# PaddlePaddle/PGL

Hardware: AMD Instinct MI355X
Metric: aggregated edges/sec (GCN send+recv_sum, d=128) (higher is better)
Workload: dtype f32

## Files before the change

pgl_amd/csrc/aggregate.hip:

```cpp
#include "aggregate_flat.hpp"
#include "aggregate_dense2.hpp"

namespace pglamd {

int chunk_edges() {
    static int k = [] {
        const char* s = getenv("PGLAMD_CHUNK");
        int v = s ? atoi(s) : 256;
        if (v < 8) v = 8;
        return v / 8 * 8;
    }();
    return k;
}

int chunk_edges_for(int64_t num_edges) {
    if (getenv("PGLAMD_CHUNK")) return chunk_edges();
    return num_edges >= 12000000 ? 256 : num_edges >= 5000000 ? 128 : 64;
}

ProfileState& prof() { static ProfileState s; return s; }

int32_t launch_fixup_cols(const AggParams& p, int32_t dtype, int rcls, hipStream_t st) {
#define PGLAMD_FIXUP(T) (rcls == 0 ? launch_fixups<T, 1, 1, 0>(p, st) : launch_fixups<T, 1, 1, 1>(p, st))
    switch (dtype) {
// ... 57 lines not shown
    PGLAMD_LAUNCH_CHECK();
    return PGLAMD_OK;
}

template int32_t aggregate_typed<float>(PGLAMD_AGG_ARGS);
extern template int32_t aggregate_typed<double>(PGLAMD_AGG_ARGS);
extern template int32_t aggregate_typed<int32_t>(PGLAMD_AGG_ARGS);
extern template int32_t aggregate_typed<int64_t>(PGLAMD_AGG_ARGS);
extern template int32_t aggregate_typed<__half>(PGLAMD_AGG_ARGS);
extern template int32_t aggregate_typed<__hip_bfloat16>(PGLAMD_AGG_ARGS);

}

using namespace pglamd;

extern "C" size_t pglamd_aggregate_workspace_bytes(int64_t num_edges, int64_t dout, int32_t dtype) {
    size_t es = dtype_size(dtype);
    if (es == 0 || num_edges <= 0) return 256;
    int64_t k = chunk_edges_for(num_edges);
    if ((int64_t)(dout * (int64_t)es) <= group_row_bytes()) k = std::min<int64_t>(k, group_chunk_edges(16));
    const int64_t n_chunks = ceil_div(num_edges, k);
    const int64_t max_cols = 1024;
    const int64_t tile = dout < max_cols ? dout : max_cols;
    if (es == 2) es = 4;
    return SplitWs(n_chunks, tile, es).bytes() + 256;
}

static int32_t aggregate_entry(const void* x, int32_t dtype, int64_t dx, const void* y, int64_t dy, const int32_t* eid,
                               const int32_t* row, const int32_t* col, const int64_t* indptr, int64_t num_edges,
                               int64_t n_csr_rows, int64_t out_rows, int64_t dout, int32_t message_op, int32_t reduce_op,
                               const float* src_scale, const float* dst_scale, int32_t accumulate, void* out, void* workspace,
                               size_t workspace_bytes, const AggExtra& ex, void* stream) {
    if (!out || !indptr || (num_edges > 0 && (!x || !row))) return fail(PGLAMD_E_ARG, "aggregate: NULL pointer");
    if (num_edges < 0 || num_edges > kMaxEdges || n_csr_rows >= INT32_MAX || out_rows >= INT32_MAX)
        return fail(PGLAMD_E_RANGE, "aggregate: sizes beyond int32 engine range");
    if (dout <= 0 || dx <= 0 || dout % dx != 0 || (y && (dy <= 0 || dout % dy != 0)))
        return fail(PGLAMD_E_SHAPE, "aggregate: dx=%lld dy=%lld dout=%lld is not a trailing-dim broadcast",
                    (long long)dx, (long long)dy, (long long)dout);
    if (reduce_op < 0 || reduce_op > 3 || (y && (message_op < 0 || message_op > 3)))
        return fail(PGLAMD_E_ARG, "aggregate: bad op enum");
    if (ex.x2 && (ex.x_split < 0 || ex.x_split >= INT32_MAX)) return fail(PGLAMD_E_RANGE, "aggregate_ext: x_split out of range");
    hipStream_t st = static_cast<hipStream_t>(stream);
#define CALL(T) aggregate_typed<T>(x, dx, y, dy, eid, row, col, indptr, num_edges, n_csr_rows, out_rows, dout, \
                                   message_op, reduce_op, src_scale, dst_scale, accumulate, out, workspace, workspace_bytes, ex, st)
    switch (dtype) {
        case PGLAMD_F32: return CALL(float);
        case PGLAMD_F64: return CALL(double);
        case PGLAMD_I32: return CALL(int32_t);
        case PGLAMD_I64: return CALL(int64_t);
        case PGLAMD_F16: return CALL(__half);
        case PGLAMD_BF16: return CALL(__hip_bfloat16);
        default: return fail(PGLAMD_E_DTYPE, "aggregate: dtype %d not supported", dtype);
    }
#undef CALL
}

extern "C" int32_t pglamd_aggregate(const void* x, int32_t dtype, int64_t n_x_rows, int64_t dx, const void* y,
                                    int64_t dy, const int32_t* eid, const int32_t* row, const int32_t* col,
                                    const int64_t* indptr, int64_t num_edges, int64_t n_csr_rows,
                                    int64_t out_rows, int64_t dout, int32_t message_op, int32_t reduce_op,
                                    const float* src_scale, const float* dst_scale, int32_t accumulate, void* out,
                                    void* workspace, size_t workspace_bytes, void* stream) {
    (void)n_x_rows;
    return aggregate_entry(x, dtype, dx, y, dy, eid, row, col, indptr, num_edges, n_csr_rows, out_rows, dout, message_op, reduce_op,
                           src_scale, dst_scale, accumulate, out, workspace, workspace_bytes, AggExtra{}, stream);
}

extern "C" int32_t pglamd_aggregate_ext(const void* x, const void* x2, int64_t x_split, int32_t dtype, int64_t dx, int64_t ldx,
                                        const void* y, int64_t dy, const int32_t* eid, const int32_t* row, const int32_t* col,
                                        const int64_t* indptr, const int64_t* zero_indptr, int64_t max_row_edges,
                                        int64_t num_edges, int64_t n_csr_rows, int64_t out_rows, int64_t dout, int64_t ldout,
                                        int32_t message_op, int32_t reduce_op, const float* dst_scale, int32_t accumulate,
                                        void* out, void* workspace, size_t workspace_bytes, int32_t flags, void* stream) {
    if (ldx < 0 || ldout < 0) return fail(PGLAMD_E_ARG, "aggregate_ext: negative row stride");
    if (flags & ~PGLAMD_AGG_DEAL_CHUNKS) return fail(PGLAMD_E_ARG, "aggregate_ext: unknown flag bits 0x%x", (unsigned)flags);
    AggExtra ex;
    ex.x2 = x2; ex.x_split = x_split; ex.zero_indptr = zero_indptr; ex.max_row_edges = max_row_edges; ex.ldx = ldx; ex.ldo = ldout;
    ex.flags = flags;
    return aggregate_entry(x, dtype, dx, y, dy, eid, row, col, indptr, num_edges, n_csr_rows, out_rows, dout, message_op, reduce_op,
                           nullptr, dst_scale, accumulate, out, workspace, workspace_bytes, ex, stream);
}

namespace pglamd {
template <int VEC>
__global__ __launch_bounds__(kBlock) void agg_slice_combine_kernel(const int* __restrict__ long_rows, int n_long, const float* __restrict__ part,
                                                                  float* __restrict__ out, int d) {
    using V = VecT<float, VEC>;
    const int lane = threadIdx.x & (kWave - 1);
    const int i = wave_uniform((int)blockIdx.x * kWavesPerBlock + (threadIdx.x >> 6));
    if (i >= n_long) return;
    const int r = as_const(long_rows)[i];
    for (int j = lane * VEC; j < d; j += kWave * VEC) {
        float* dst = out + (int64_t)r * d + j;
        V acc = *reinterpret_cast<const V*>(dst);
        V v[kXcds];
#pragma unroll
        for (int s = 0; s < kXcds; ++s) v[s] = *reinterpret_cast<const V*>(part + ((int64_t)s * n_long + i) * d + j);
#pragma unroll
        for (int k = 0; k < VEC; ++k) {
            double a = acc.v[k];
#pragma unroll
            for (int s = 0; s < kXcds; ++s) a += (double)v[s].v[k];
            acc.v[k] = (float)a;
        }
        *reinterpret_cast<V*>(dst) = acc;
    }
}

struct SlicedWs {
    size_t table, part;
    SplitWs split;
    SlicedWs(int64_t n_chunks, int64_t d, int64_t n_hubs, int64_t n_long)
        : table(align_up((size_t)n_hubs * d * sizeof(float), 256)), part(align_up((size_t)kXcds * n_long * d * sizeof(float), 256)),
          split(n_chunks, d, sizeof(float)) {}
    size_t bytes() const { return table + part + split.bytes(); }
};
}

extern "C" size_t pglamd_aggregate_sliced_workspace_bytes(int64_t num_edges, int64_t d, int64_t n_hubs, int64_t n_long, int32_t chunk) {
    if (num_edges <= 0 || d <= 0 || n_hubs < 0 || n_long < 0 || chunk < 8) return 256;
    return SlicedWs(ceil_div(num_edges, chunk), d, n_hubs, n_long).bytes() + 256;
}

extern "C" int32_t pglamd_aggregate_sliced(const float* x, int64_t n_x_rows, int64_t d, const int32_t* hub_ids, int64_t n_hubs,
                                           const int32_t* row, const int32_t* col, const int64_t* indptr, int64_t num_edges,
                                           int64_t out_rows, const int32_t* long_rows, int64_t n_long, const int32_t* blocks,
                                           const int32_t* blocks_dev, int32_t chunk, float* out, void* workspace,
                                           size_t workspace_bytes, void* stream) {
    if (!x || !hub_ids || !row || !col || !indptr || !long_rows || !blocks || !blocks_dev || !out || !workspace)
        return fail(PGLAMD_E_ARG, "aggregate_sliced: NULL pointer");
    const int64_t n_rows = out_rows + kXcds * n_long;
    if (num_edges <= 0 || num_edges > kMaxEdges || n_x_rows <= 0 || n_hubs <= 0 || n_long <= 0 || out_rows <= 0 ||
        n_rows >= INT32_MAX || n_x_rows + n_hubs >= INT32_MAX)
        return fail(PGLAMD_E_RANGE, "aggregate_sliced: sizes beyond int32 engine range");
    if (chunk < 8 || chunk % 8 != 0) return fail(PGLAMD_E_ARG, "aggregate_sliced: chunk %d is not a positive multiple of 8", (int)chunk);
    const int vec = (d % 4 == 0 && d > 128) ? 4 : 2;
    if (d % vec != 0 || d / vec > kWave) return fail(PGLAMD_E_SHAPE, "aggregate_sliced: d = %lld is not an even width up to 128 or a multiple of 4 up to 256", (long long)d);
    if ((reinterpret_cast<uintptr_t>(x) | reinterpret_cast<uintptr_t>(out) | reinterpret_cast<uintptr_t>(workspace)) % (vec * sizeof(float)) != 0)
        return fail(PGLAMD_E_ARG, "aggregate_sliced: x / out / workspace must be %d-byte aligned", (int)(vec * sizeof(float)));
    const int64_t n_chunks = ceil_div(num_edges, chunk), nb = ceil_div(n_chunks, kWavesPerBlock);
    for (int s = 0; s <= kXcds; ++s) {
        const int64_t end = s < kXcds ? blocks[s + 1] : nb;
        if (blocks[s] < 0 || blocks[kXcds + 1 + s] < 0 || (int64_t)blocks[s] + blocks[kXcds + 1 + s] != end || (s == 0 && blocks[0] != 0))
            return fail(PGLAMD_E_ARG, "aggregate_sliced: block table does not tile the %lld blocks of the stream (segment %d)", (long long)nb, s);
    }
    const SlicedWs lay(n_chunks, d, n_hubs, n_long);
    if (workspace_bytes < lay.bytes() + 256) return fail(PGLAMD_E_WORKSPACE, "aggregate_sliced: workspace %zu < %zu", workspace_bytes, lay.bytes() + 256);
    hipStream_t st = static_cast<hipStream_t>(stream);
    char* ws = static_cast<char*>(workspace);
    float* table = reinterpret_cast<float*>(ws);
    float* part = reinterpret_cast<float*>(ws + lay.table);
    PGLAMD_TRY(pglamd_gather_rows(x, d, sizeof(float), hub_ids, 0, n_hubs, table, stream));
    AggParams p{};
    p.x = x; p.x2 = table - n_x_rows * d; p.x_split = (int)n_x_rows;
    p.out = out; p.pout = part - out_rows * d; p.slice_tab = blocks_dev;
    p.row = row; p.col = col; p.indptr = indptr; p.zero_indptr = indptr;
    p.ldx = d; p.ldo = d; p.out_rows = out_rows; p.n_csr_rows = n_rows; p.E = (int)num_edges;
    p.gy = 1; p.j_base = 0; p.tile_cols = (int)d; p.zvec = vec; p.align = 1;
    p.chunk = chunk; p.n_chunks = (int)n_chunks;
    lay.split.carve(p, ws + lay.table + lay.part);
    const int64_t per_xcd = slice_blocks_per_xcd(blocks);
    PGLAMD_TRY(vec == 4 ? launch_flat_sliced<4>(p, per_xcd, st) : launch_flat_sliced<2>(p, per_xcd, st));
    const unsigned grid = (unsigned)ceil_div(n_long, kWavesPerBlock);
    if (vec == 4) hipLaunchKernelGGL(agg_slice_combine_kernel<4>, dim3(grid), dim3(kBlock), 0, st, long_rows, (int)n_long, part, out, (int)d);
    else hipLaunchKernelGGL(agg_slice_combine_kernel<2>, dim3(grid), dim3(kBlock), 0, st, long_rows, (int)n_long, part, out, (int)d);
    PGLAMD_LAUNCH_CHECK();
    return PGLAMD_OK;
}

namespace pglamd {
__global__ __launch_bounds__(kBlock) void pack_weight_kernel(const float* __restrict__ w, int d_in, int d_out, float* __restrict__ wp) {
    const int KK = d_in / 4;
    const int64_t total = (int64_t)(d_out / 16) * KK * kWave;
    for (int64_t i = (int64_t)blockIdx.x * kBlock + threadIdx.x; i < total; i += (int64_t)gridDim.x * kBlock) {
        const int lane = (int)(i % kWave);
        const int64_t t = i / kWave;
        const int kk = (int)(t % KK), ct = (int)(t / KK);
        wp[i] = w[(int64_t)(4 * kk + lane / 16) * d_out + ct * 16 + (lane & 15)];
    }
}

template <int VEC, int SS = 0>
static int32_t launch_dense(AggParams p, hipStream_t st) {
    const int64_t nb = ceil_div(p.n_chunks, kWavesPerBlock);
    p.n_blocks = (int)nb;
    p.n_grid_chunks = (int)xcd_grid(nb);
    const int64_t zb = ceil_div(ceil_div(p.out_rows, kWave), kWavesPerBlock);
    const bool fixups = needs_fixups(p);
    if (fixups) PGLAMD_TRY(reset_split_counters(p, st));
    ProfileScope timed(st, [] { return std::string("agg_flat_kernel<float, ") + (VEC == 2 ? "2" : "1") + ", 1, 0, 0, dense sink>"; });
    hipLaunchKernelGGL((agg_flat_kernel<float, VEC, 1, 0, 0, SS, true, 0, 1>), dim3((unsigned)(p.n_grid_chunks + zb)), dim3(kBlock), 0, st, p);
    PGLAMD_LAUNCH_CHECK();
    PGLAMD_TRY(timed.close());
    if (!fixups) return PGLAMD_OK;
    PGLAMD_TRY((launch_fixups<float, VEC, 1, 0>(p, st)));
    return launch_dense_hub<VEC>(p, st);
}
}

extern "C" size_t pglamd_aggregate_dense_workspace_bytes(int64_t num_edges, int64_t d_in, int64_t d_out) {
    return pglamd_aggregate_workspace_bytes(num_edges, d_in, PGLAMD_F32) + align_up((size_t)(d_in > 0 ? d_in : 1) * (size_t)(d_out > 0 ? d_out : 1) * 4, 256) + 256;
}

extern "C" int32_t pglamd_aggregate_dense(const float* x, int64_t d_in, const int32_t* row, const int32_t* col, const int64_t* indptr,
                                          int64_t num_edges, int64_t n_csr_rows, int64_t out_rows, int32_t reduce_op,
                                          const float* edge_scale, const float* dst_scale, const float* w, const float* bias, int32_t act,
                                          int64_t d_out, float* agg_out, float* out, void* workspace, size_t workspace_bytes, void* stream) {
    if (!out || !w || !indptr || (num_edges > 0 && (!x || !row || !col))) return fail(PGLAMD_E_ARG, "aggregate_dense: NULL pointer");
    if (num_edges < 0 || num_edges > kMaxEdges || n_csr_rows >= INT32_MAX || out_rows >= INT32_MAX)
        return fail(PGLAMD_E_RANGE, "aggregate_dense: sizes beyond int32 engine range");
    if ((d_in != 64 && d_in != 128) || d_out <= 0 || d_out % 16 != 0 || d_out > 1024)
        return fail(PGLAMD_E_SHAPE, "aggregate_dense: d_in must be 64 or 128 and d_out a multiple of 16 up to 1024 (got %lld, %lld)", (long long)d_in, (long long)d_out);
    if (reduce_op != PGLAMD_SUM && reduce_op != PGLAMD_MEAN) return fail(PGLAMD_E_ARG, "aggregate_dense: sum or mean");
    if ((reinterpret_cast<uintptr_t>(x) | reinterpret_cast<uintptr_t>(agg_out) | reinterpret_cast<uintptr_t>(workspace)) % 8 != 0)
        return fail(PGLAMD_E_ARG, "aggregate_dense: x / agg_out / workspace must be 8-byte aligned");
    if (!workspace || workspace_bytes < pglamd_aggregate_dense_workspace_bytes(num_edges, d_in, d_out))
        return fail(PGLAMD_E_WORKSPACE, "aggregate_dense: workspace too small");
    if (out_rows == 0) return PGLAMD_OK;
    hipStream_t st = static_cast<hipStream_t>(stream);
    float* wp = static_cast<float*>(workspace);
    const size_t wp_bytes = align_up((size_t)d_in * (size_t)d_out * 4, 256);
    static const int form_env = [] { const char* e = getenv("PGLAMD_DENSE_FORM"); return e ? atoi(e) : 0; }();
    const bool form2 = form_env != 1 && dense2_covers(d_in, d_out) && reinterpret_cast<uintptr_t>(w) % 16 == 0;
    if (form_env == 2 && !form2) return fail(PGLAMD_E_SHAPE, "aggregate_dense: form 2 needs d_in * d_out * 4 + ring <= 80 KB");
    {
        const int64_t total = form2 ? d_in * d_out : (d_out / 16) * (d_in / 4) * kWave;
        const unsigned grid = (unsigned)std::min<int64_t>(ceil_div(total, kBlock), 1024);
        if (!form2) {
            hipLaunchKernelGGL(pack_weight_kernel, dim3(grid), dim3(kBlock), 0, st, w, (int)d_in, (int)d_out, wp);
            PGLAMD_LAUNCH_CHECK();
        }
    }
    char* ws = static_cast<char*>(workspace) + wp_bytes;
    AggParams p{};
    p.x = x; p.x2 = x; p.x_split = INT32_MAX; p.out = agg_out; p.row = row; p.col = col; p.indptr = indptr; p.zero_indptr = indptr;
    p.dst_scale = dst_scale;
    p.src_scale = edge_scale; p.ss_by_pos = edge_scale ? 1 : 0;
    p.ldx = d_in; p.ldo = d_in; p.out_rows = out_rows; p.n_csr_rows = n_csr_rows; p.E = (int)num_edges;
    p.is_mean = reduce_op == PGLAMD_MEAN; p.gy = 1;
    p.w = w; p.wp = wp; p.bias = bias; p.out2 = out; p.dout2 = (int)d_out; p.act = act;
    p.j_base = 0; p.tile_cols = (int)d_in; p.zvec = 2; p.align = 1;
    const int K = chunk_edges_for(num_edges);
    p.chunk = K;
    p.n_chunks = (int)ceil_div(num_edges > 0 ? num_edges : 1, (int64_t)K);
    SplitWs(p.n_chunks, d_in, sizeof(float)).carve(p, ws);
    if (num_edges == 0) p.n_chunks = 0;
// ... 41 lines not shown
```

pgl_amd/csrc/aggregate.hpp:

```cpp
#pragma once
#include <atomic>
#include <mutex>
#include "common.hpp"
#include "split_rows.hpp"

#include <string>
#include <type_traits>
#include <utility>
#include <vector>

namespace pglamd {

struct AggParams {
    const void* x; const void* y; void* out;
    const void* x2;
    const int64_t* zero_indptr;
    const int* row; const int* col; const int* eid;
    const int64_t* indptr;
    const float* src_scale; const float* dst_scale;
    int ss_by_pos;
    void* part_head; void* part_tail;
    int* long_count; int* long_list;
    int* long_list2;
    int64_t ldx, ldy, ldo;
    int64_t out_rows, n_csr_rows;
    int E, n_chunks, chunk, n_blocks;
    int n_grid_chunks;
    int j_base, tile_cols;
    int gy;
    int ypad;
    int mop, is_max, is_mean;
    int zvec;
    int accumulate;
    int align;
    int narrow_vec;
    int x_split;
    int deal_chunks;
    const float* w;
    const float* wp;
    const float* bias;
    float* out2;
    int dout2, act;
    int max_row_edges;
    const int* slice_tab;
    void* pout;
};

inline bool needs_fixups(const AggParams& p) {
    return p.n_chunks > 1 && !(p.align && p.max_row_edges > 0 && p.max_row_edges <= p.chunk);
}

template <typename T, int VEC> struct alignas(sizeof(T) * VEC) VecT { T v[VEC]; };

template <typename T> struct AccT { using type = T; };
template <> struct AccT<__half> { using type = float; };
template <> struct AccT<__hip_bfloat16> { using type = float; };
template <typename T> __device__ __forceinline__ typename AccT<T>::type to_acc(T v) { return v; }
template <> __device__ __forceinline__ float to_acc<__half>(__half v) { return __half2float(v); }
template <> __device__ __forceinline__ float to_acc<__hip_bfloat16>(__hip_bfloat16 v) { return __bfloat162float(v); }
template <typename T> __device__ __forceinline__ T from_acc(typename AccT<T>::type v) { return v; }
template <> __device__ __forceinline__ __half from_acc<__half>(float v) { return __float2half(v); }
template <> __device__ __forceinline__ __hip_bfloat16 from_acc<__hip_bfloat16>(float v) { return __float2bfloat16(v); }

template <typename T> struct Limits;
template <> struct Limits<float> { static __device__ float lo() { return -INFINITY; } static __device__ float hi() { return INFINITY; } };
template <> struct Limits<double> { static __device__ double lo() { return -INFINITY; } static __device__ double hi() { return INFINITY; } };
template <> struct Limits<int32_t> { static __device__ int32_t lo() { return INT32_MIN; } static __device__ int32_t hi() { return INT32_MAX; } };
template <> struct Limits<int64_t> { static __device__ int64_t lo() { return INT64_MIN; } static __device__ int64_t hi() { return INT64_MAX; } };

template <typename A> __device__ __forceinline__ A nan_max(A a, A b) {
    if constexpr (std::is_floating_point_v<A>) return __builtin_elementwise_maximum(a, b);
    else return a > b ? a : b;
}
template <typename A> __device__ __forceinline__ A nan_min(A a, A b) {
    if constexpr (std::is_floating_point_v<A>) return __builtin_elementwise_minimum(a, b);
    else return a < b ? a : b;
}

template <typename T> __device__ __forceinline__ T apply_mop(T a, T b, int mop) {
    switch (mop) {
        case PGLAMD_ADD: return a + b;
        case PGLAMD_SUB: return a - b;
        case PGLAMD_MUL: return a * b;
        default: return a / b;
    }
}

template <typename T, bool SLICED = false>
__device__ __forceinline__ void zero_empty_rows_role(const AggParams& p, int64_t zb, int lane) {
    const int64_t w = zb * kWavesPerBlock + (threadIdx.x >> 6);
    const int64_t r0 = w * kWave;
    const int64_t n_rows = SLICED ? p.n_csr_rows : p.out_rows;
    if (r0 >= n_rows) return;
    const int64_t r = r0 + lane;
    bool empty = false;
    if (r < n_rows) empty = (r >= p.n_csr_rows) || (p.zero_indptr[r] == p.zero_indptr[r + 1]);
    unsigned long long m = __ballot(empty);
    T* out = static_cast<T*>(p.out) + p.j_base;
    while (m) {
        const int l = __builtin_ctzll(m);
        m &= m - 1;
        T* dst = out + (r0 + l) * p.ldo;
        if constexpr (SLICED) { if (r0 + l >= p.out_rows) dst = static_cast<T*>(p.pout) + p.j_base + (r0 + l) * p.ldo; }
        if (p.zvec == 4) {
            for (int j = lane * 4; j < p.tile_cols; j += kWave * 4) *reinterpret_cast<VecT<T, 4>*>(dst + j) = VecT<T, 4>{};
        } else if (p.zvec == 2) {
            for (int j = lane * 2; j < p.tile_cols; j += kWave * 2) *reinterpret_cast<VecT<T, 2>*>(dst + j) = VecT<T, 2>{};
        } else {
            for (int j = lane; j < p.tile_cols; j += kWave) dst[j] = from_acc<T>(typename AccT<T>::type(0));
        }
    }
}

__device__ __forceinline__ void dense_empty_rows_role(const AggParams& p, int64_t zb, int lane) {
    const int64_t w = zb * kWavesPerBlock + (threadIdx.x >> 6);
    const int64_t r0 = w * kWave;
    if (r0 >= p.out_rows) return;
    const int64_t r = r0 + lane;
    bool empty = false;
    if (r < p.out_rows) empty = (r >= p.n_csr_rows) || (p.zero_indptr[r] == p.zero_indptr[r + 1]);
    unsigned long long m = __ballot(empty);
    while (m) {
        const int l = __builtin_ctzll(m);
        m &= m - 1;
        float* dst = p.out2 + (r0 + l) * (int64_t)p.dout2;
        for (int j = lane; j < p.dout2; j += kWave) {
            float v = p.bias ? p.bias[j] : 0.f;
            if (p.act) v = relu_f(v);
            dst[j] = v;
        }
    }
}

struct ProfileState {
    std::atomic<bool> on{false};
    std::mutex mu;
    std::string last_kernel;
    std::vector<std::pair<hipEvent_t, hipEvent_t>> ev;
};
ProfileState& prof();

class ProfileScope {
    hipStream_t st_;
    hipEvent_t e0_ = nullptr, e1_ = nullptr;
    int32_t rc_ = PGLAMD_OK;
    int32_t open() {
        PGLAMD_HIP_CHECK(hipEventCreate(&e0_));
        PGLAMD_HIP_CHECK(hipEventCreate(&e1_));
        PGLAMD_HIP_CHECK(hipEventRecord(e0_, st_));
        return PGLAMD_OK;
    }
public:
    template <typename F> ProfileScope(hipStream_t st, F&& kernel_name) : st_(st) {
        if (!prof().on.load(std::memory_order_relaxed)) return;
        { std::lock_guard<std::mutex> lk(prof().mu); prof().last_kernel = kernel_name(); }
        rc_ = open();
    }
    int32_t close() {
        if (!e1_ || rc_ != PGLAMD_OK) return rc_;
        PGLAMD_HIP_CHECK(hipEventRecord(e1_, st_));
        std::lock_guard<std::mutex> lk(prof().mu);
        prof().ev.emplace_back(e0_, e1_);
        return PGLAMD_OK;
    }
};

int narrow_chunk_edges();
int32_t launch_fixup_cols(const AggParams& p, int32_t dtype, int rcls, hipStream_t st);
int32_t launch_narrow(const AggParams& p, int32_t dtype, int rcls, int64_t dy, hipStream_t st, bool* handled);

bool narrow_softmax_covers(int64_t d, int32_t dtype);
size_t narrow_softmax_workspace_bytes(int64_t num_rows, int64_t d, int32_t dtype, int chunk);
int32_t narrow_softmax_stats(const void* data, int32_t dtype, int64_t num_rows, int64_t d, const int32_t* row32,
                             const int32_t* perm32, const int64_t* seg_ptr, int64_t n_seg, void* stats,
                             int chunk, void* ws, size_t ws_bytes, hipStream_t st);

}
```

pgl_amd/csrc/aggregate_flat.hpp:

```cpp
#pragma once
#include "aggregate.hpp"
#include "aggregate_group.hpp"

#include <algorithm>
#include <string>
#include <type_traits>
#include <utility>
#include <vector>

namespace pglamd {

int narrow_max();
int32_t zero_empty_rows(const int64_t* indptr, int64_t n_csr_rows, int64_t out_rows, void* out, size_t row_bytes, hipStream_t st);


template <typename T, int VEC, int NT, int RCLS, int YMODE, int SS = 0, bool PIPE3 = true, int UB = 0, int SINK = 0, bool TWO = false, bool SLICED = false>
__global__ __launch_bounds__(kBlock) void agg_flat_kernel(AggParams p) {
    constexpr int U = 8;
    constexpr int kTileRows = 16;
    constexpr int kTileStride = kWave * VEC + 4;
    static_assert(SINK == 0 || (std::is_same_v<T, float> && NT == 1 && RCLS == 0 && YMODE == 0 && UB == 0 && (VEC == 1 || VEC == 2)),
                  "the dense sink takes fp32 rows of 64 or 128 columns");
    static_assert(!SLICED || (std::is_same_v<T, float> && NT == 1 && RCLS == 0 && YMODE == 0 && SS == 0 && SINK == 0 && TWO),
                  "hub slices: plain fp32 sums of one tile over two source tables");
    using V = VecT<T, VEC>;
    using A = typename AccT<T>::type;
    using VA = VecT<A, VEC>;
    const int lane = threadIdx.x & (kWave - 1);
    const int wib = wave_uniform(threadIdx.x >> 6);
    if ((int)blockIdx.x >= p.n_grid_chunks) {
        if constexpr (SINK == 1) {
            if (p.out) zero_empty_rows_role<T>(p, (int64_t)blockIdx.x - p.n_grid_chunks, lane);
            dense_empty_rows_role(p, (int64_t)blockIdx.x - p.n_grid_chunks, lane);
        } else {
            zero_empty_rows_role<T, SLICED>(p, (int64_t)blockIdx.x - p.n_grid_chunks, lane);
        }
        return;
    }
    int64_t lb;
    if constexpr (SLICED) lb = slice_block(as_const(p.slice_tab), blockIdx.x);
    else lb = xcd_swizzle(blockIdx.x, p.n_blocks);
    if (lb < 0) return;
    const int c = wave_uniform((int)lb * kWavesPerBlock + wib);
    if (c >= p.n_chunks) return;
    const cptr<int> rowp = as_const(p.row);
    const cptr<int> colp = as_const(p.col);
    const int e0 = p.align ? chunk_cut(rowp, as_const(p.indptr), c * p.chunk, p.chunk, p.E) : c * p.chunk;
    const int e1 = p.align ? chunk_cut(rowp, as_const(p.indptr), c * p.chunk + p.chunk, p.chunk, p.E) : min(c * p.chunk + p.chunk, p.E);
    if (e0 >= e1) return;
    const cptr<int> eidp = as_const(p.eid);
    const T* __restrict__ x = static_cast<const T*>(p.x);
    const T* __restrict__ y = static_cast<const T*>(p.y);
    const T* __restrict__ x2 = static_cast<const T*>(p.x2);
    const int xs = p.x_split;
    auto src_row = [&](int cc) -> const T* {
        if constexpr (TWO) return (cc < xs ? x : x2) + (int64_t)cc * p.ldx;
        else return x + (int64_t)cc * p.ldx;
    };
    constexpr bool has_ss = SS != 0;
    const bool is_max = p.is_max != 0;

    int j0[NT]; bool act[NT];
#pragma unroll
    for (int t = 0; t < NT; ++t) {
        j0[t] = (t * kWave + lane) * VEC;
        act[t] = j0[t] < p.tile_cols;
        j0[t] += p.j_base;
    }

    int yj[NT];
#pragma unroll
    for (int t = 0; t < NT; ++t) yj[t] = (YMODE == 1 || YMODE == 3) ? j0[t] / p.gy : 0;

    A acc[NT][VEC];
    double accd[SLICED ? NT : 1][SLICED ? VEC : 1];
    auto reset = [&]() {
#pragma unroll
        for (int t = 0; t < NT; ++t)
#pragma unroll
            for (int k = 0; k < VEC; ++k) {
                acc[t][k] = RCLS == 0 ? A(0) : Limits<A>::lo();
                if constexpr (SLICED) accd[t][k] = 0.0;
            }
    };
    reset();
    auto fold = [&]() {
        if constexpr (SLICED) {
#pragma unroll
            for (int t = 0; t < NT; ++t)
#pragma unroll
                for (int k = 0; k < VEC; ++k) acc[t][k] = (A)accd[t][k];
        }
    };
    const bool neg = RCLS == 1 && !is_max;

    int cur = rowp[e0];
    bool head_open = e0 > 0 && rowp[e0 - 1] == cur;

    const cptr<AggParams> kargs = (cptr<AggParams>)__builtin_amdgcn_kernarg_segment_ptr();
    auto cold = [&]() -> cptr<AggParams> {
        cptr<AggParams> q = kargs;
        asm volatile("" : "+s"(q));
        return q;
    };
    float (*sink_tile)[kTileRows][kTileStride] = nullptr;
    int (*sink_rows)[kTileRows] = nullptr;
    if constexpr (SINK == 1) {
        __shared__ float st[kWavesPerBlock][kTileRows][kTileStride];
        __shared__ int sr[kWavesPerBlock][kTileRows];
        sink_tile = st; sink_rows = sr;
    }
    int n_parked = 0;
    auto flush_tile = [&]() {
        if constexpr (SINK == 1) {
            const cptr<AggParams> q = cold();
            constexpr int KK = kWave * VEC / 4;
            __builtin_amdgcn_fence(__ATOMIC_RELEASE, "wavefront");
            __builtin_amdgcn_wave_barrier();
            float a[KK];
            const float* trow = &sink_tile[wib][lane & 15][lane >> 4];
#pragma unroll
            for (int kk = 0; kk < KK; ++kk) a[kk] = trow[4 * kk];
            const float* __restrict__ wp = q->wp;
// ... 19 lines not shown
                    if (rr < n_parked) {
                        float v = acc4[i] + bv;
                        if (relu) v = relu_f(v);
                        out2[(int64_t)sink_rows[wib][rr] * ldo2 + colj] = v;
                    }
                }
            }
            __builtin_amdgcn_wave_barrier();
            n_parked = 0;
        }
    };
    auto store_partial = [&](bool head) {
        fold();
        const cptr<AggParams> q = cold();
        A* dst = static_cast<A*>(head ? q->part_head : q->part_tail) + (int64_t)c * q->tile_cols;
        const int jb = q->j_base;
#pragma unroll
        for (int t = 0; t < NT; ++t)
            if (act[t]) {
                VA o;
#pragma unroll
                for (int k = 0; k < VEC; ++k) o.v[k] = RCLS == 1 ? order_flip(acc[t][k], neg) : acc[t][k];
                *reinterpret_cast<VA*>(dst + (j0[t] - jb)) = o;
            }
        if (!head && lane == 0) {
            if constexpr (SINK == 0) {
                const int b = chunk_of_edge(as_const(q->indptr)[cur + 1] - 1, q->chunk);
                const bool lng = fixup_is_long(c, b);
                (lng ? q->long_list2 : q->long_list)[atomicAdd(q->long_count + (lng ? 1 : 0), 1)] = c;
            } else {
                q->long_list[atomicAdd(q->long_count, 1)] = c;
            }
        }
    };
    auto store_final = [&](int r) {
        fold();
        const cptr<AggParams> q = cold();
        T* dst;
        if constexpr (SLICED) {
            dst = (r >= q->out_rows ? static_cast<T*>(q->pout) : static_cast<T*>(q->out)) + (int64_t)r * q->ldo;
        } else {
            if (r >= q->out_rows) return;
            dst = static_cast<T*>(q->out) + (int64_t)r * q->ldo;
        }
        const float* dsp = q->dst_scale;
        const bool is_mean = q->is_mean != 0, accumulate = q->accumulate == 1;
        float ds = 1.f;
        int64_t n = 1;
        if constexpr (RCLS == 0) {
            if (dsp) ds = as_const(dsp)[r];
            if (is_mean) { const cptr<int64_t> ipq = as_const(q->indptr); n = ipq[r + 1] - ipq[r]; }
        }
#pragma unroll
        for (int t = 0; t < NT; ++t)
            if (act[t]) {
                A ov[VEC];
#pragma unroll
                for (int k = 0; k < VEC; ++k) {
                    A a = RCLS == 1 ? order_flip(acc[t][k], neg) : acc[t][k];
                    if constexpr (RCLS == 0) {
                        if (is_mean) a = a / (A)n;
                        if constexpr (std::is_floating_point_v<A>) { if (dsp) a = a * (A)ds; }
                    }
                    ov[k] = a;
                }
                if (accumulate) {
                    const V old = *reinterpret_cast<const V*>(dst + j0[t]);
#pragma unroll
                    for (int k = 0; k < VEC; ++k) {
                        const A ol = to_acc<T>(old.v[k]);
                        if constexpr (RCLS == 0) ov[k] = ol + ov[k];
                        else ov[k] = is_max ? nan_max(ov[k], ol) : nan_min(ov[k], ol);
                    }
                }
                V o;
#pragma unroll
                for (int k = 0; k < VEC; ++k) o.v[k] = from_acc<T>(ov[k]);
                if constexpr (SINK == 1) {
                    float* tr = &sink_tile[wib][n_parked][0];
#pragma unroll
                    for (int k = 0; k < VEC; ++k) tr[j0[t] - q->j_base + k] = (float)ov[k];
                    if (q->out) *reinterpret_cast<V*>(dst + j0[t]) = o;
                } else {
                    *reinterpret_cast<V*>(dst + j0[t]) = o;
                }
            }
        if constexpr (SINK == 1) {
            if (lane == 0) sink_rows[wib][n_parked] = r;
            if (++n_parked == kTileRows) flush_tile();
        }
    };
    auto flush_mid = [&]() {
        if (head_open) store_partial(true); else store_final(cur);
        head_open = false;
    };

    const float* __restrict__ sscale_v = p.src_scale;
    const int* __restrict__ col_v = p.col;
    auto scale_of = [&](int col) -> float {
        int ci = col;
        asm volatile("" : "+v"(ci));
        return sscale_v[ci];
    };
    auto load_idx = [&](int e, int (&cc)[U], int (&rr)[U], int (&yy)[U]) {
#pragma unroll
        for (int i = 0; i < U; ++i) {
            rr[i] = rowp[e + i];
            cc[i] = colp ? colp[e + i] : e + i;
            if constexpr (YMODE == 1 || YMODE == 2) yy[i] = eidp ? eidp[e + i] : e + i;
        }
    };
    auto load_cl = [&](int e, int& cl) {
        if constexpr (SS == 2) cl = e + (lane & (U - 1));
        else if constexpr (has_ss) cl = col_v ? col_v[e + (lane & (U - 1))] : e + (lane & (U - 1));
    };
    const int* __restrict__ eid_v = p.eid;
    const int ypad = YMODE == 3 ? p.ypad : 1;
    const int y_edge = lane / ypad, y_elem = lane % ypad;
    const bool y_lane = YMODE == 3 && y_edge < U && y_elem < (int)p.ldy;
    auto load_yl = [&](int e, int& yl) {
        if constexpr (YMODE == 3) { if (y_lane) yl = eid_v ? eid_v[e + y_edge] : e + y_edge; }
    };
    auto load_yv = [&](int yl, T& yv) {
        if constexpr (YMODE == 3) { if (y_lane) yv = y[(int64_t)yl * p.ldy + y_elem]; }
    };
    auto load_rows = [&](const int (&cc)[U], const int (&yy)[U], V (&vx)[U][NT], V (&vy)[U][NT], int cl, float& sv) {
        if constexpr (has_ss) sv = sscale_v[cl];
#pragma unroll
        for (int i = 0; i < U; ++i) {
            const T* xr = src_row(cc[i]);
#pragma unroll
            for (int t = 0; t < NT; ++t)
                if (act[t]) vx[i][t] = *reinterpret_cast<const V*>(xr + j0[t]);
            if constexpr (YMODE == 1) {
                const T* yr = y + (int64_t)yy[i] * p.ldy;
#pragma unroll
                for (int t = 0; t < NT; ++t)
                    if (act[t]) vy[i][t].v[0] = yr[yj[t]];
            } else if constexpr (YMODE == 2) {
                const T* yr = y + (int64_t)yy[i] * p.ldy;
#pragma unroll
                for (int t = 0; t < NT; ++t)
                    if (act[t]) vy[i][t] = *reinterpret_cast<const V*>(yr + j0[t]);
            }
        }
    };
    auto consume_one = [&](int r, float s, const V (&vx)[NT], const V (&vy)[NT], T ys = T{}) {
        if (r != cur) { flush_mid(); cur = r; reset(); }
#pragma unroll
        for (int t = 0; t < NT; ++t)
#pragma unroll
            for (int k = 0; k < VEC; ++k) {
                A m = to_acc<T>(vx[t].v[k]);
                if constexpr (std::is_floating_point_v<A>) { if (has_ss) m = m * (A)s; }
                if constexpr (YMODE == 1) m = apply_mop(m, to_acc<T>(vy[t].v[0]), p.mop);
                if constexpr (YMODE == 2) m = apply_mop(m, to_acc<T>(vy[t].v[k]), p.mop);
                if constexpr (YMODE == 3) m = apply_mop(m, to_acc<T>(ys), p.mop);
                if constexpr (SLICED) accd[t][k] += (double)m;
                else if constexpr (RCLS == 0) acc[t][k] += m;
                else acc[t][k] = max_of(acc[t][k], order_flip(m, neg));
            }
    };
    auto lane_scale = [&](float sv, int i) -> float {
        if constexpr (has_ss) return __int_as_float(__builtin_amdgcn_readlane(__float_as_int(sv), i));
        else return 1.f;
    };

// ... 359 lines not shown
            if (t > s) out[j] = from_acc<T>(additive ? ol + acc : (p.is_max == 1 ? nan_max(acc, ol) : nan_min(acc, ol)));
        } else if (p.accumulate == 2) {
            if (t > s) out[j] = from_acc<T>(acc);
        } else {
            out[j] = from_acc<T>(acc);
        }
    }
}

template <typename T> const char* type_name() {
    return std::is_same_v<T, float> ? "float" : std::is_same_v<T, double> ? "double" : std::is_same_v<T, int32_t> ? "int" :
           std::is_same_v<T, int64_t> ? "long" : std::is_same_v<T, __half> ? "__half" : "__hip_bfloat16";
}
template <typename T> std::string kernel_name(int vec, int nt, int rcls, int ymode) {
    char b[96];
    snprintf(b, sizeof(b), "agg_flat_kernel<%s, %d, %d, %d, %d>", type_name<T>(), vec, nt, rcls, ymode);
    return b;
}

template <typename T, int VEC, int NT, int RCLS, int YMODE>
int32_t launch_flat(AggParams p, hipStream_t st) {
    const int64_t nb = ceil_div(p.n_chunks, kWavesPerBlock);
    static const bool env_off = [] { const char* sw = getenv("PGLAMD_XCD_SWIZZLE"); return sw && sw[0] == '0'; }();
    p.n_blocks = (env_off || p.deal_chunks) ? -(int)nb : (int)nb;
    p.n_grid_chunks = (int)xcd_grid(nb);
    const int64_t zb = p.accumulate ? 0 : ceil_div(ceil_div(p.out_rows, kWave), kWavesPerBlock);
    const bool fixups = needs_fixups(p);
    if (fixups) PGLAMD_TRY(reset_split_counters(p, st));
    ProfileScope timed(st, [] { return kernel_name<T>(VEC, NT, RCLS, YMODE); });
    constexpr bool can_scale = RCLS == 0 && std::is_floating_point_v<typename AccT<T>::type>;
    const size_t row_bytes = (size_t)p.tile_cols * sizeof(T);
    const bool two = p.x_split != INT32_MAX;
#define PGLAMD_LAUNCH_FLAT(...)                                                                                                          \
    do {                                                                                                                                 \
        const dim3 grid_((unsigned)(p.n_grid_chunks + zb));                                                                              \
        if (two) hipLaunchKernelGGL((agg_flat_kernel<T, VEC, NT, RCLS, YMODE, __VA_ARGS__, 0, true>), grid_, dim3(kBlock), 0, st, p);      \
        else hipLaunchKernelGGL((agg_flat_kernel<T, VEC, NT, RCLS, YMODE, __VA_ARGS__, 0, false>), grid_, dim3(kBlock), 0, st, p);         \
        PGLAMD_LAUNCH_CHECK();                                                                                                           \
    } while (0)
    if constexpr (NT == 1 && YMODE == 0) {
        static const int vidx_max = [] { const char* e = getenv("PGLAMD_VIDX_BYTES"); return e ? atoi(e) : 320; }();
        if ((int)row_bytes <= vidx_max && !p.src_scale) {
            PGLAMD_LAUNCH_FLAT(false, true, 16);
            goto launched;
        }
        if (row_bytes >= 192 && row_bytes <= 320 && !p.src_scale) {
            PGLAMD_LAUNCH_FLAT(false, false, 0);
            goto launched;
        }
    }
    if constexpr (can_scale) {
        if (p.src_scale) {
            bool by_pos = false;
            if constexpr (std::is_same_v<T, float> && YMODE == 0) {
                if (p.ss_by_pos) {
                    by_pos = true;
                    if (two) hipLaunchKernelGGL((agg_flat_kernel<T, VEC, NT, RCLS, YMODE, 2, true, 0, 0, true>), dim3((unsigned)(p.n_grid_chunks + zb)), dim3(kBlock), 0, st, p);
                    else hipLaunchKernelGGL((agg_flat_kernel<T, VEC, NT, RCLS, YMODE, 2>), dim3((unsigned)(p.n_grid_chunks + zb)), dim3(kBlock), 0, st, p);
                }
            }
            if (!by_pos) hipLaunchKernelGGL((agg_flat_kernel<T, VEC, NT, RCLS, YMODE, 1>), dim3((unsigned)(p.n_grid_chunks + zb)), dim3(kBlock), 0, st, p);
            PGLAMD_LAUNCH_CHECK();
        } else {
            PGLAMD_LAUNCH_FLAT(false, true, 0);
        }
    } else {
        PGLAMD_LAUNCH_FLAT(false, true, 0);
    }
#undef PGLAMD_LAUNCH_FLAT
launched:
    PGLAMD_TRY(timed.close());
    if (fixups) {
        const unsigned gl = fixup_grid_long(p.n_chunks), gs = fixup_grid_short(p.n_chunks, kFixGridMergedShort, kFixWaves);
        hipLaunchKernelGGL((agg_fixup_merged_kernel<T, VEC, NT, RCLS>), dim3(gl + gs), dim3(kFixWaves * kWave), 0, st, p, (int)gl);
    }
    PGLAMD_LAUNCH_CHECK();
    return PGLAMD_OK;
}

template <int VEC>
int32_t launch_flat_sliced(AggParams p, int64_t blocks_per_xcd, hipStream_t st) {
    p.n_blocks = (int)ceil_div(p.n_chunks, kWavesPerBlock);
    p.n_grid_chunks = (int)(blocks_per_xcd * kXcds);
    const int64_t zb = ceil_div(ceil_div(p.n_csr_rows, kWave), kWavesPerBlock);
    PGLAMD_TRY(reset_split_counters(p, st));
    ProfileScope timed(st, [] { return kernel_name<float>(VEC, 1, 0, 0) + " hub slices"; });
    hipLaunchKernelGGL((agg_flat_kernel<float, VEC, 1, 0, 0, 0, true, 0, 0, true, true>), dim3((unsigned)(p.n_grid_chunks + zb)), dim3(kBlock), 0, st, p);
    PGLAMD_LAUNCH_CHECK();
    PGLAMD_TRY(timed.close());
    const unsigned gl = fixup_grid_long(p.n_chunks), gs = fixup_grid_short(p.n_chunks, kFixGridMergedShort, kFixWaves);
    hipLaunchKernelGGL((agg_fixup_merged_kernel<float, VEC, 1, 0, true>), dim3(gl + gs), dim3(kFixWaves * kWave), 0, st, p, (int)gl);
    PGLAMD_LAUNCH_CHECK();
    return PGLAMD_OK;
}

template <typename T> constexpr int32_t dtype_code() {
    return std::is_same_v<T, float> ? PGLAMD_F32 : std::is_same_v<T, double> ? PGLAMD_F64 : std::is_same_v<T, int32_t> ? PGLAMD_I32 :
           std::is_same_v<T, int64_t> ? PGLAMD_I64 : std::is_same_v<T, __half> ? PGLAMD_F16 : PGLAMD_BF16;
}

template <typename T, int VEC, int NT>
int32_t dispatch_mode(const AggParams& p, int rcls, int ymode, hipStream_t st, bool* handled) {
    *handled = true;
    if (rcls == 0) {
        if (ymode == 0) return launch_flat<T, VEC, NT, 0, 0>(p, st);
        if constexpr (std::is_floating_point_v<T>) {
            if constexpr (NT == 1) { if (ymode == 1 && p.ypad > 0) return launch_flat<T, VEC, NT, 0, 3>(p, st); }
            if (ymode == 1) return launch_flat<T, VEC, NT, 0, 1>(p, st);
            if (ymode == 2) return launch_flat<T, VEC, NT, 0, 2>(p, st);
        }
    } else if (ymode == 0) {
        return launch_flat<T, VEC, NT, 1, 0>(p, st);
    }
    *handled = false;
    return PGLAMD_OK;
}

template <typename T> constexpr int max_vec() { return sizeof(T) == 2 ? 8 : sizeof(T) == 4 ? 4 : 2; }
template <typename T> constexpr int max_tiles(int vec) { return (sizeof(T) == 2 && vec == 8) ? 2 : 4; }

template <typename T, int VEC>
int32_t dispatch_tiles(const AggParams& p, int rcls, int ymode, hipStream_t st, bool* handled) {
    const int64_t tiles = ceil_div(p.tile_cols, kWave * VEC);
    if (tiles <= 1) return dispatch_mode<T, VEC, 1>(p, rcls, ymode, st, handled);
    if constexpr (max_tiles<T>(VEC) >= 4) {
        if (tiles > 2) return dispatch_mode<T, VEC, 4>(p, rcls, ymode, st, handled);
    }
    return dispatch_mode<T, VEC, 2>(p, rcls, ymode, st, handled);
}

template <typename T>
int32_t dispatch_shape(const AggParams& p, int vec, int rcls, int ymode, hipStream_t st, bool* handled) {
    if constexpr (max_vec<T>() >= 8) { if (vec >= 8) return dispatch_tiles<T, 8>(p, rcls, ymode, st, handled); }
    if constexpr (max_vec<T>() >= 4) { if (vec >= 4) return dispatch_tiles<T, 4>(p, rcls, ymode, st, handled); }
    if (vec >= 2) return dispatch_tiles<T, 2>(p, rcls, ymode, st, handled);
    return dispatch_tiles<T, 1>(p, rcls, ymode, st, handled);
}

struct AggExtra {
    const void* x2 = nullptr; int64_t x_split = 0; const int64_t* zero_indptr = nullptr; int64_t max_row_edges = 0;
    int64_t ldx = 0, ldo = 0;
    int32_t flags = 0;
};

#define PGLAMD_AGG_ARGS const void*, int64_t, const void*, int64_t, const int32_t*, const int32_t*, const int32_t*, const int64_t*, \
                        int64_t, int64_t, int64_t, int64_t, int32_t, int32_t, const float*, const float*, int, void*, void*, size_t, \
                        const AggExtra&, hipStream_t

template <typename T>
int32_t aggregate_typed(const void* x, int64_t dx, const void* y, int64_t dy, const int32_t* eid,
                               const int32_t* row, const int32_t* col, const int64_t* indptr, int64_t E,
                               int64_t n_csr_rows, int64_t out_rows, int64_t dout, int32_t mop, int32_t rop,
                               const float* src_scale, const float* dst_scale, int accumulate, void* out, void* ws,
                               size_t ws_bytes, const AggExtra& ex, hipStream_t st) {
    int32_t rc = PGLAMD_OK;
    if (accumulate && rop == PGLAMD_MEAN)
        return fail(PGLAMD_E_ARG, "aggregate: accumulate with MEAN is undefined (use SUM with dst_scale = 1/degree)");
    const int64_t* zip = ex.zero_indptr ? ex.zero_indptr : indptr;
    const int64_t ldx = ex.ldx ? ex.ldx : dx, ldo = ex.ldo ? ex.ldo : dout;
    if (ldx < dx || ldo < dout) return fail(PGLAMD_E_SHAPE, "aggregate_ext: row stride shorter than the row (ldx %lld < %lld or ldout %lld < %lld)",
                                            (long long)ldx, (long long)dx, (long long)ldo, (long long)dout);
    if (E == 0) {
        if (accumulate) return PGLAMD_OK;
        if (ldo != dout) return fail(PGLAMD_E_ARG, "aggregate_ext: an index without edges cannot zero-fill a strided output");
        return zero_empty_rows(zip, n_csr_rows, out_rows, out, (size_t)dout * sizeof(T), st);
    }

    AggParams p{};
// ... 107 lines not shown
```

pgl_amd/csrc/common.cpp:

```cpp
#include "common.hpp"
#include <atomic>

namespace pglamd {

std::string& last_error_ref() {
    thread_local std::string e;
    return e;
}

int32_t fail(int32_t code, const char* fmt, ...) {
    char buf[512];
    va_list ap;
    va_start(ap, fmt);
    vsnprintf(buf, sizeof(buf), fmt, ap);
    va_end(ap);
    last_error_ref() = buf;
    return code;
}

std::atomic<int>& csr_onesweep_option() {
    static std::atomic<int> v{[] { const char* e = getenv("PGLAMD_CSR_ONESWEEP"); return e ? atoi(e) : -1; }()};
    return v;
}

}

extern "C" int32_t pglamd_abi_version(void) { return PGLAMD_ABI_VERSION; }

extern "C" int32_t pglamd_set_option(const char* name, int64_t value) {
    if (!name) return pglamd::fail(PGLAMD_E_ARG, "set_option: NULL name");
    if (strcmp(name, "csr_onesweep") == 0) { pglamd::csr_onesweep_option().store(value < -1 ? -1 : value > 64 ? 64 : (int)value, std::memory_order_relaxed); return PGLAMD_OK; }
    return pglamd::fail(PGLAMD_E_ARG, "set_option: unknown option %s", name);
}

extern "C" const char* pglamd_last_error(void) { return pglamd::last_error_ref().c_str(); }

extern "C" const char* pglamd_device_arch(void) {
    thread_local std::string arch;
    int dev = 0;
    hipDeviceProp_t prop;
    if (hipGetDevice(&dev) != hipSuccess || hipGetDeviceProperties(&prop, dev) != hipSuccess) {
        (void)hipGetLastError();
        arch = "";
        return arch.c_str();
    }
    arch = prop.gcnArchName;
    return arch.c_str();
}
```

pgl_amd/csrc/common.hpp:

```cpp
#pragma once
#include <hip/hip_runtime.h>
#include <hip/hip_fp16.h>
#include <hip/hip_bf16.h>

#include <algorithm>
#include <atomic>
#include <cstdarg>
#include <cstring>
#include <cstdlib>
#include <cstdint>
#include <cstdio>
#include <string>

#include "../../include/pgl_amd.h"

namespace pglamd {

constexpr int kWave = 64;
constexpr int kBlock = 256;
constexpr int kWavesPerBlock = kBlock / kWave;
constexpr int kXcds = 8;
constexpr int64_t kMaxEdges = (int64_t)INT32_MAX - 65536;

std::string& last_error_ref();
int32_t fail(int32_t code, const char* fmt, ...);

#define PGLAMD_HIP_CHECK(expr)                                                             \
    do {                                                                                   \
        hipError_t _e = (expr);                                                            \
        if (_e != hipSuccess)                                                              \
            return ::pglamd::fail(PGLAMD_E_HIP, "%s failed: %s (%s:%d)", #expr,            \
                                  hipGetErrorString(_e), __FILE__, __LINE__);              \
    } while (0)

#define PGLAMD_LAUNCH_CHECK() PGLAMD_HIP_CHECK(hipGetLastError())

#define PGLAMD_TRY(expr)                                                                   \
    do {                                                                                   \
        const int32_t _rc = (expr);                                                        \
        if (_rc != PGLAMD_OK) return _rc;                                                  \
    } while (0)

inline size_t align_up(size_t x, size_t a) { return (x + a - 1) / a * a; }
inline int64_t ceil_div(int64_t a, int64_t b) { return (a + b - 1) / b; }

inline size_t dtype_size(int32_t dt) {
    switch (dt) {
        case PGLAMD_F16: case PGLAMD_BF16: return 2;
        case PGLAMD_F32: case PGLAMD_I32: return 4;
        case PGLAMD_F64: case PGLAMD_I64: return 8;
        default: return 0;
    }
}

struct Carver {
    char* base; size_t cap; size_t off = 0;
    Carver(void* p, size_t n) : base(static_cast<char*>(p)), cap(n) {}
    template <typename T> T* take(size_t count) {
        size_t bytes = align_up(count * sizeof(T), 256);
        T* r = reinterpret_cast<T*>(base + off);
        off += bytes;
        return r;
    }
    bool ok() const { return base != nullptr && off <= cap; }
};

__device__ __forceinline__ int64_t xcd_swizzle(int64_t b, int64_t nb) {
    if (nb < 0) return b < -nb ? b : -1;
    int64_t per = (nb + kXcds - 1) / kXcds;
    int64_t lb = (b % kXcds) * per + b / kXcds;
    return lb < nb ? lb : -1;
}
inline int64_t xcd_grid(int64_t nb) { return ceil_div(nb, kXcds) * kXcds; }
std::atomic<int>& csr_onesweep_option();

__device__ __forceinline__ int wave_uniform(int v) { return __builtin_amdgcn_readfirstlane(v); }

template <typename T> using cptr = const T __attribute__((address_space(4)))*;
template <typename T> __device__ __forceinline__ cptr<T> as_const(const T* p) {
    return (cptr<T>)(unsigned long long)p;
}

__device__ __forceinline__ int chunk_cut(cptr<int> rowp, cptr<int64_t> ip, int pos, int K, int E) {
    if (pos <= 0) return 0;
    if (pos >= E) return E;
    const int r = rowp[pos];
    const int64_t rs = ip[r];
    if (rs == pos) return pos;
    const int64_t re = ip[r + 1];
    if (re - rs > K) return pos;
    return (int)re;
}

__host__ __device__ __forceinline__ int slice_rest_lo(int n_rest, int x) { return (int)((int64_t)n_rest * x / kXcds); }
__device__ __forceinline__ int64_t slice_block(cptr<int> tab, int64_t b) {
    const int x = (int)(b % kXcds), j = (int)(b / kXcds);
    const int n_rest = tab[kXcds + 1];
    const int r_lo = slice_rest_lo(n_rest, x), nr = slice_rest_lo(n_rest, x + 1) - r_lo;
    const int ns = tab[kXcds + 2 + x], s_lo = tab[1 + x];
    const int total = nr + ns;
    if (j >= total) return -1;
    const int a = (int)((int64_t)j * ns / total);
    return (int)((int64_t)(j + 1) * ns / total) > a ? s_lo + a : r_lo + (j - a);
}
inline int64_t slice_blocks_per_xcd(const int* tab) {
    int64_t m = 0;
    for (int x = 0; x < kXcds; ++x)
        m = std::max<int64_t>(m, slice_rest_lo(tab[kXcds + 1], x + 1) - slice_rest_lo(tab[kXcds + 1], x) + tab[kXcds + 2 + x]);
    return m;
}

__device__ __forceinline__ float relu_f(float v) { return v < 0.f ? 0.f : v; }

}
```

Before: 20.65 billion.

## Fuse hub gather with counter reset, batch combine rows, stream partial stores

Replaces the generic hub-row gather with a dedicated wide-word gather kernel that also zeroes the split counters, which removes the separate counter-reset launch. The combine kernel now handles two long rows per wave and issues all partial loads before the accumulate. Stores to the per-XCD partial buffer in the sliced path become nontemporal. A tunable 'slice_front' option is added that controls how slice blocks are interleaved with the remaining blocks; its default of 100 keeps the previous interleaving. The combine kernel now assumes d fits in a single pass of one wave.

Result: faster. 21.62 billion, median of 6 (+4.7%).

```diff
diff --git a/pgl_amd/csrc/aggregate.hip b/pgl_amd/csrc/aggregate.hip
--- a/pgl_amd/csrc/aggregate.hip
+++ b/pgl_amd/csrc/aggregate.hip
@@ -163,29 +163,64 @@
 }
 
 namespace pglamd {
+template <typename W>
+__global__ __launch_bounds__(kBlock) void gather_hubs_kernel(const W* __restrict__ x, int64_t row_words, const int* __restrict__ hub_ids,
+                                                             int64_t n_hubs, W* __restrict__ table, int* __restrict__ counts) {
+    if (blockIdx.x == 0 && threadIdx.x == 0) { counts[kSplitCountList1] = 0; counts[kSplitCountList2] = 0; }
+    const int64_t total = n_hubs * row_words;
+    for (int64_t i = (int64_t)blockIdx.x * kBlock + threadIdx.x; i < total; i += (int64_t)gridDim.x * kBlock) {
+        const int64_t r = i / row_words, w = i - r * row_words;
+        table[i] = x[(int64_t)hub_ids[r] * row_words + w];
+    }
+}
+
+template <typename W>
+static int32_t gather_hubs(const float* x, int64_t d, const int32_t* hub_ids, int64_t n_hubs, float* table, int* counts, hipStream_t st) {
+    const int64_t rw = d * (int64_t)sizeof(float) / (int64_t)sizeof(W);
+    const unsigned grid = (unsigned)std::min<int64_t>(ceil_div(n_hubs * rw, kBlock), 256 * 32);
+    hipLaunchKernelGGL(gather_hubs_kernel<W>, dim3(grid), dim3(kBlock), 0, st, reinterpret_cast<const W*>(x), rw, hub_ids, n_hubs,
+                       reinterpret_cast<W*>(table), counts);
+    PGLAMD_LAUNCH_CHECK();
+    return PGLAMD_OK;
+}
+
+constexpr int kCombineRows = 2;
 template <int VEC>
 __global__ __launch_bounds__(kBlock) void agg_slice_combine_kernel(const int* __restrict__ long_rows, int n_long, const float* __restrict__ part,
                                                                   float* __restrict__ out, int d) {
     using V = VecT<float, VEC>;
     const int lane = threadIdx.x & (kWave - 1);
-    const int i = wave_uniform((int)blockIdx.x * kWavesPerBlock + (threadIdx.x >> 6));
-    if (i >= n_long) return;
-    const int r = as_const(long_rows)[i];
-    for (int j = lane * VEC; j < d; j += kWave * VEC) {
-        float* dst = out + (int64_t)r * d + j;
-        V acc = *reinterpret_cast<const V*>(dst);
-        V v[kXcds];
-#pragma unroll
-        for (int s = 0; s < kXcds; ++s) v[s] = *reinterpret_cast<const V*>(part + ((int64_t)s * n_long + i) * d + j);
-#pragma unroll
-        for (int k = 0; k < VEC; ++k) {
-            double a = acc.v[k];
-#pragma unroll
-            for (int s = 0; s < kXcds; ++s) a += (double)v[s].v[k];
-            acc.v[k] = (float)a;
+    const int i0 = wave_uniform(((int)blockIdx.x * kWavesPerBlock + (threadIdx.x >> 6)) * kCombineRows);
+    if (i0 >= n_long) return;
+    const int j = lane * VEC;
+    if (j >= d) return;
+    const int n = min(kCombineRows, n_long - i0);
+    V acc[kCombineRows], v[kCombineRows][kXcds];
+    float* dst[kCombineRows];
+#pragma unroll
+    for (int q = 0; q < kCombineRows; ++q)
+        if (q < n) {
+#pragma unroll
+            for (int s = 0; s < kXcds; ++s) v[q][s] = *reinterpret_cast<const V*>(part + ((int64_t)s * n_long + i0 + q) * d + j);
         }
-        *reinterpret_cast<V*>(dst) = acc;
-    }
+#pragma unroll
+    for (int q = 0; q < kCombineRows; ++q)
+        if (q < n) {
+            dst[q] = out + (int64_t)as_const(long_rows)[i0 + q] * d + j;
+            acc[q] = *reinterpret_cast<const V*>(dst[q]);
+        }
+#pragma unroll
+    for (int q = 0; q < kCombineRows; ++q)
+        if (q < n) {
+#pragma unroll
+            for (int k = 0; k < VEC; ++k) {
+                double a = acc[q].v[k];
+#pragma unroll
+                for (int s = 0; s < kXcds; ++s) a += (double)v[q][s].v[k];
+                acc[q].v[k] = (float)a;
+            }
+            *reinterpret_cast<V*>(dst[q]) = acc[q];
+        }
 }
 
 struct SlicedWs {
@@ -231,7 +266,6 @@
     char* ws = static_cast<char*>(workspace);
     float* table = reinterpret_cast<float*>(ws);
     float* part = reinterpret_cast<float*>(ws + lay.table);
-    PGLAMD_TRY(pglamd_gather_rows(x, d, sizeof(float), hub_ids, 0, n_hubs, table, stream));
     AggParams p{};
     p.x = x; p.x2 = table - n_x_rows * d; p.x_split = (int)n_x_rows;
     p.out = out; p.pout = part - out_rows * d; p.slice_tab = blocks_dev;
@@ -240,9 +274,11 @@
     p.gy = 1; p.j_base = 0; p.tile_cols = (int)d; p.zvec = vec; p.align = 1;
     p.chunk = chunk; p.n_chunks = (int)n_chunks;
     lay.split.carve(p, ws + lay.table + lay.part);
+    const bool w16 = d % 4 == 0 && (reinterpret_cast<uintptr_t>(x) | reinterpret_cast<uintptr_t>(table)) % 16 == 0;
+    PGLAMD_TRY(w16 ? gather_hubs<uint4>(x, d, hub_ids, n_hubs, table, p.long_count, st) : gather_hubs<uint2>(x, d, hub_ids, n_hubs, table, p.long_count, st));
     const int64_t per_xcd = slice_blocks_per_xcd(blocks);
     PGLAMD_TRY(vec == 4 ? launch_flat_sliced<4>(p, per_xcd, st) : launch_flat_sliced<2>(p, per_xcd, st));
-    const unsigned grid = (unsigned)ceil_div(n_long, kWavesPerBlock);
+    const unsigned grid = (unsigned)ceil_div(n_long, kCombineRows * kWavesPerBlock);
     if (vec == 4) hipLaunchKernelGGL(agg_slice_combine_kernel<4>, dim3(grid), dim3(kBlock), 0, st, long_rows, (int)n_long, part, out, (int)d);
     else hipLaunchKernelGGL(agg_slice_combine_kernel<2>, dim3(grid), dim3(kBlock), 0, st, long_rows, (int)n_long, part, out, (int)d);
     PGLAMD_LAUNCH_CHECK();
diff --git a/pgl_amd/csrc/aggregate.hpp b/pgl_amd/csrc/aggregate.hpp
--- a/pgl_amd/csrc/aggregate.hpp
+++ b/pgl_amd/csrc/aggregate.hpp
@@ -44,6 +44,7 @@
     int max_row_edges;
     const int* slice_tab;
     void* pout;
+    int slice_front;
 };
 
 inline bool needs_fixups(const AggParams& p) {
@@ -51,6 +52,18 @@
 }
 
 template <typename T, int VEC> struct alignas(sizeof(T) * VEC) VecT { T v[VEC]; };
+
+template <bool STREAM, typename V> __device__ __forceinline__ void row_store(V* p, const V& v) {
+    if constexpr (STREAM && sizeof(V) == 16) {
+        typedef unsigned u4 __attribute__((ext_vector_type(4)));
+        __builtin_nontemporal_store(*reinterpret_cast<const u4*>(&v), reinterpret_cast<u4*>(p));
+    } else if constexpr (STREAM && sizeof(V) == 8) {
+        typedef unsigned u2 __attribute__((ext_vector_type(2)));
+        __builtin_nontemporal_store(*reinterpret_cast<const u2*>(&v), reinterpret_cast<u2*>(p));
+    } else {
+        *p = v;
+    }
+}
 
 template <typename T> struct AccT { using type = T; };
 template <> struct AccT<__half> { using type = float; };
@@ -103,9 +116,9 @@
         T* dst = out + (r0 + l) * p.ldo;
         if constexpr (SLICED) { if (r0 + l >= p.out_rows) dst = static_cast<T*>(p.pout) + p.j_base + (r0 + l) * p.ldo; }
         if (p.zvec == 4) {
-            for (int j = lane * 4; j < p.tile_cols; j += kWave * 4) *reinterpret_cast<VecT<T, 4>*>(dst + j) = VecT<T, 4>{};
+            for (int j = lane * 4; j < p.tile_cols; j += kWave * 4) row_store<SLICED>(reinterpret_cast<VecT<T, 4>*>(dst + j), VecT<T, 4>{});
         } else if (p.zvec == 2) {
-            for (int j = lane * 2; j < p.tile_cols; j += kWave * 2) *reinterpret_cast<VecT<T, 2>*>(dst + j) = VecT<T, 2>{};
+            for (int j = lane * 2; j < p.tile_cols; j += kWave * 2) row_store<SLICED>(reinterpret_cast<VecT<T, 2>*>(dst + j), VecT<T, 2>{});
         } else {
             for (int j = lane; j < p.tile_cols; j += kWave) dst[j] = from_acc<T>(typename AccT<T>::type(0));
         }
diff --git a/pgl_amd/csrc/aggregate_flat.hpp b/pgl_amd/csrc/aggregate_flat.hpp
--- a/pgl_amd/csrc/aggregate_flat.hpp
+++ b/pgl_amd/csrc/aggregate_flat.hpp
@@ -38,7 +38,7 @@
         return;
     }
     int64_t lb;
-    if constexpr (SLICED) lb = slice_block(as_const(p.slice_tab), blockIdx.x);
+    if constexpr (SLICED) lb = slice_block(as_const(p.slice_tab), blockIdx.x, p.slice_front);
     else lb = xcd_swizzle(blockIdx.x, p.n_blocks);
     if (lb < 0) return;
     const int c = wave_uniform((int)lb * kWavesPerBlock + wib);
@@ -224,7 +224,7 @@
                     for (int k = 0; k < VEC; ++k) tr[j0[t] - q->j_base + k] = (float)ov[k];
                     if (q->out) *reinterpret_cast<V*>(dst + j0[t]) = o;
                 } else {
-                    *reinterpret_cast<V*>(dst + j0[t]) = o;
+                    row_store<SLICED>(reinterpret_cast<V*>(dst + j0[t]), o);
                 }
             }
         if constexpr (SINK == 1) {
@@ -750,8 +750,8 @@
 int32_t launch_flat_sliced(AggParams p, int64_t blocks_per_xcd, hipStream_t st) {
     p.n_blocks = (int)ceil_div(p.n_chunks, kWavesPerBlock);
     p.n_grid_chunks = (int)(blocks_per_xcd * kXcds);
+    p.slice_front = slice_front_option().load(std::memory_order_relaxed);
     const int64_t zb = ceil_div(ceil_div(p.n_csr_rows, kWave), kWavesPerBlock);
-    PGLAMD_TRY(reset_split_counters(p, st));
     ProfileScope timed(st, [] { return kernel_name<float>(VEC, 1, 0, 0) + " hub slices"; });
     hipLaunchKernelGGL((agg_flat_kernel<float, VEC, 1, 0, 0, 0, true, 0, 0, true, true>), dim3((unsigned)(p.n_grid_chunks + zb)), dim3(kBlock), 0, st, p);
     PGLAMD_LAUNCH_CHECK();
diff --git a/pgl_amd/csrc/common.cpp b/pgl_amd/csrc/common.cpp
--- a/pgl_amd/csrc/common.cpp
+++ b/pgl_amd/csrc/common.cpp
@@ -23,6 +23,15 @@
     return v;
 }
 
+int slice_front_default() {
+    static const int d = [] { const char* e = getenv("PGLAMD_SLICE_FRONT"); const int v = e ? atoi(e) : kSliceFrontDefault; return v < 0 ? 0 : v > 100 ? 100 : v; }();
+    return d;
+}
+std::atomic<int>& slice_front_option() {
+    static std::atomic<int> v{slice_front_default()};
+    return v;
+}
+
 }
 
 extern "C" int32_t pglamd_abi_version(void) { return PGLAMD_ABI_VERSION; }
@@ -30,6 +39,7 @@
 extern "C" int32_t pglamd_set_option(const char* name, int64_t value) {
     if (!name) return pglamd::fail(PGLAMD_E_ARG, "set_option: NULL name");
     if (strcmp(name, "csr_onesweep") == 0) { pglamd::csr_onesweep_option().store(value < -1 ? -1 : value > 64 ? 64 : (int)value, std::memory_order_relaxed); return PGLAMD_OK; }
+    if (strcmp(name, "slice_front") == 0) { pglamd::slice_front_option().store(value < 0 ? pglamd::slice_front_default() : value > 100 ? 100 : (int)value, std::memory_order_relaxed); return PGLAMD_OK; }
     return pglamd::fail(PGLAMD_E_ARG, "set_option: unknown option %s", name);
 }
 
diff --git a/pgl_amd/csrc/common.hpp b/pgl_amd/csrc/common.hpp
--- a/pgl_amd/csrc/common.hpp
+++ b/pgl_amd/csrc/common.hpp
@@ -93,16 +93,21 @@
 }
 
 __host__ __device__ __forceinline__ int slice_rest_lo(int n_rest, int x) { return (int)((int64_t)n_rest * x / kXcds); }
-__device__ __forceinline__ int64_t slice_block(cptr<int> tab, int64_t b) {
+__device__ __forceinline__ int64_t slice_block(cptr<int> tab, int64_t b, int front) {
     const int x = (int)(b % kXcds), j = (int)(b / kXcds);
     const int n_rest = tab[kXcds + 1];
     const int r_lo = slice_rest_lo(n_rest, x), nr = slice_rest_lo(n_rest, x + 1) - r_lo;
     const int ns = tab[kXcds + 2 + x], s_lo = tab[1 + x];
     const int total = nr + ns;
     if (j >= total) return -1;
-    const int a = (int)((int64_t)j * ns / total);
-    return (int)((int64_t)(j + 1) * ns / total) > a ? s_lo + a : r_lo + (j - a);
+    const int head = max(ns, min(total, (int)(((int64_t)total * front + 99) / 100)));
+    if (j >= head) return r_lo + (j - ns);
+    const int a = (int)((int64_t)j * ns / head);
+    return (int)((int64_t)(j + 1) * ns / head) > a ? s_lo + a : r_lo + (j - a);
 }
+constexpr int kSliceFrontDefault = 100;
+int slice_front_default();
+std::atomic<int>& slice_front_option();
 inline int64_t slice_blocks_per_xcd(const int* tab) {
     int64_t m = 0;
     for (int x = 0; x < kXcds; ++x)
```
